# JokerYan/MS-GS

Measured on AMD Instinct MI355X. Metric: Mpixels/s fwd+bwd @1080p, 1M Gaussians; fraction of HBM roofline, higher is better.
Workload: dtype f32

## Files before the change

### ms-gs_amd/csrc/preprocess.hip

```cpp
#include "msgs_internal.h"

#include <type_traits>

#pragma clang fp contract(off)

namespace msgs {

namespace {

constexpr float SH_C0 = 0.28209479177387814f;
constexpr float SH_C1 = 0.4886025119029199f;
__device__ constexpr float SH_C2[5] = {1.0925484305920792f, -1.0925484305920792f, 0.31539156525252005f,
                                       -1.0925484305920792f, 0.5462742152960396f};
__device__ constexpr float SH_C3[7] = {-0.5900435899266435f, 2.890611442640554f, -0.4570457994644658f,
                                       0.3731763325901154f, -0.4570457994644658f, 1.445305721320277f,
                                       -0.5900435899266435f};

struct Cam {
    float V[16];
    float M[16];
    float cam[3];
};

__device__ __forceinline__ void load_cam(const ViewParams& vp, Cam& c) {
// ... 99 lines not shown
    float r = SH_C0 * S(0);
    if (deg > 0) {
        r = r - SH_C1 * y * S(1) + SH_C1 * z * S(2) - SH_C1 * x * S(3);
        if (deg > 1) {
            const float xx = x * x, yy = y * y, zz = z * z, xy = x * y, yz = y * z, xz = x * z;
            r = r + SH_C2[0] * xy * S(4) + SH_C2[1] * yz * S(5) + SH_C2[2] * (2.0f * zz - xx - yy) * S(6) +
                SH_C2[3] * xz * S(7) + SH_C2[4] * (xx - yy) * S(8);
            if (deg > 2) {
                r = r + SH_C3[0] * y * (3.0f * xx - yy) * S(9) + SH_C3[1] * xy * z * S(10) +
                    SH_C3[2] * y * (4.0f * zz - xx - yy) * S(11) +
                    SH_C3[3] * z * (2.0f * zz - 3.0f * xx - 3.0f * yy) * S(12) +
                    SH_C3[4] * x * (4.0f * zz - xx - yy) * S(13) + SH_C3[5] * z * (xx - yy) * S(14) +
                    SH_C3[6] * x * (xx - 3.0f * yy) * S(15);
            }
        }
    }
    return r;
}


__device__ __forceinline__ void sh_basis(int deg, float x, float y, float z, float b[16]) {
#pragma unroll
    for (int k = 0; k < 16; ++k) b[k] = 0.f;
    b[0] = SH_C0;
    if (deg > 0) {
        b[1] = -(SH_C1 * y); b[2] = SH_C1 * z; b[3] = -(SH_C1 * x);
        if (deg > 1) {
            const float xx = x * x, yy = y * y, zz = z * z, xy = x * y, yz = y * z, xz = x * z;
            b[4] = SH_C2[0] * xy; b[5] = SH_C2[1] * yz; b[6] = SH_C2[2] * (2.0f * zz - xx - yy);
            b[7] = SH_C2[3] * xz; b[8] = SH_C2[4] * (xx - yy);
            if (deg > 2) {
                b[9] = SH_C3[0] * y * (3.0f * xx - yy); b[10] = SH_C3[1] * xy * z;
                b[11] = SH_C3[2] * y * (4.0f * zz - xx - yy);
                b[12] = SH_C3[3] * z * (2.0f * zz - 3.0f * xx - 3.0f * yy);
                b[13] = SH_C3[4] * x * (4.0f * zz - xx - yy); b[14] = SH_C3[5] * z * (xx - yy);
                b[15] = SH_C3[6] * x * (xx - 3.0f * yy);
            }
        }
    }
}

__device__ __forceinline__ void wave_lds_fence() {
    __builtin_amdgcn_fence(__ATOMIC_RELEASE, "wavefront");
    __builtin_amdgcn_wave_barrier();
    __builtin_amdgcn_fence(__ATOMIC_ACQUIRE, "wavefront");
}

constexpr int ROW_F = 48;
constexpr int ROW_LDS = 49;
constexpr int K9_STAGE_ROWS = 32;

__device__ __forceinline__ int sh_row_float4s(int deg) { return deg == 0 ? 1 : deg == 1 ? 3 : deg == 2 ? 7 : 12; }

__device__ __forceinline__ void coop_load_rows(float* lds_rows, const float* g_rows, const uint8_t* idx, int nrow,
                                               int n4, int lane, int row0 = 0) {
    const int rpi = 64 / n4;
    const int sub = lane / n4, c = lane - sub * n4;
    for (int it = 0; it * rpi < nrow; ++it) {
        const int slot = it * rpi + sub;
        if (sub < rpi && slot < nrow) {
            const int sl = idx[slot];
            const float4 v = *reinterpret_cast<const float4*>(g_rows + (size_t)sl * ROW_F + 4 * c);
            float* d = lds_rows + (sl - row0) * ROW_LDS + 4 * c;
            d[0] = v.x; d[1] = v.y; d[2] = v.z; d[3] = v.w;
        }
    }
}

constexpr int HALF_F4 = 6;
constexpr int HALF_LDS = 25;
__device__ __forceinline__ void coop_load_rows_part(float* lds_rows, const float* g_rows, const uint8_t* idx, int nrow,
                                                    int f4_first, int n4, int lane) {
    const int rpi = 64 / n4;
    const int sub = lane / n4, c = lane - sub * n4;
    for (int it = 0; it * rpi < nrow; ++it) {
        const int slot = it * rpi + sub;
        if (sub < rpi && slot < nrow) {
            const int sl = idx[slot];
            const float4 v = *reinterpret_cast<const float4*>(g_rows + (size_t)sl * ROW_F + 4 * (f4_first + c));
            float* d = lds_rows + sl * HALF_LDS + 4 * c;
            d[0] = v.x; d[1] = v.y; d[2] = v.z; d[3] = v.w;
        }
    }
}

__device__ __forceinline__ void coop_store_rows(const float* lds_rows, float* g_rows, int nrow, uint64_t live,
                                                int nfloat, int lane, bool acc) {
    constexpr int n4 = ROW_F / 4, rpi = 64 / n4;
    const int sub = lane / n4, c = lane - sub * n4;
    for (int it = 0; it * rpi < nrow; ++it) {
        const int row = it * rpi + sub;
        if (sub < rpi && row < nrow) {
            const bool on = (live >> row) & 1ull;
            if (acc && !on) continue;
            float4 v = make_float4(0.f, 0.f, 0.f, 0.f);
            if (on) {
                const float* sp = lds_rows + row * ROW_LDS + 4 * c;
                v.x = 4 * c + 0 < nfloat ? sp[0] : 0.f;
                v.y = 4 * c + 1 < nfloat ? sp[1] : 0.f;
                v.z = 4 * c + 2 < nfloat ? sp[2] : 0.f;
                v.w = 4 * c + 3 < nfloat ? sp[3] : 0.f;
            }
            float4* dst = reinterpret_cast<float4*>(g_rows + (size_t)row * ROW_F + 4 * c);
            if (acc) { const float4 o = *dst; v.x = o.x + v.x; v.y = o.y + v.y; v.z = o.z + v.z; v.w = o.w + v.w; }
            *dst = v;
        }
    }
}

constexpr int REST_F = 45;

__device__ __forceinline__ float act_opacity(const msgs_gaussians_t& g, int i) {
    const float x = g.opacities[i];
    return g.raw_params == 1 ? 1.0f / (1.0f + expf(-x)) : x;
}
__device__ __forceinline__ void act_scales(const msgs_gaussians_t& g, int i, float* s) {
#pragma unroll
    for (int k = 0; k < 3; ++k) { const float x = g.scales[3 * i + k]; s[k] = g.raw_params == 1 ? expf(x) : x; }
}
__device__ __forceinline__ float act_rotation(const msgs_gaussians_t& g, int i, float* q) {
    const float4 q4 = reinterpret_cast<const float4*>(g.rotations)[i];
    q[0] = q4.x; q[1] = q4.y; q[2] = q4.z; q[3] = q4.w;
    if (g.raw_params == 0) return 1.0f;
    if (g.raw_params == 2) {
        const float4 r4 = reinterpret_cast<const float4*>(g.rotations_raw)[i];
        return sqrtf(r4.x * r4.x + r4.y * r4.y + r4.z * r4.z + r4.w * r4.w);
    }
    const float rn = sqrtf(q[0] * q[0] + q[1] * q[1] + q[2] * q[2] + q[3] * q[3]);
    const float n = fmaxf(rn, 1e-12f);
#pragma unroll
    for (int k = 0; k < 4; ++k) q[k] = q[k] / n;
    return rn;
}
__device__ __forceinline__ void normalize_backward(const float* q, float rn, float* dq) {
    const float n = fmaxf(rn, 1e-12f);
    const float dotq = rn < 1e-12f ? 0.f : q[0] * dq[0] + q[1] * dq[1] + q[2] * dq[2] + q[3] * dq[3];
#pragma unroll
    for (int k = 0; k < 4; ++k) dq[k] = (dq[k] - q[k] * dotq) / n;
}

typedef float msgs_f3 __attribute__((ext_vector_type(3)));
typedef msgs_f3 __attribute__((aligned(4))) msgs_f3_u;
__device__ __forceinline__ void coop_load_split_half_listed(float* lds_rows, const float* dc, const float* rest, int wave_first,
                                                            const uint8_t* idx, int nlisted, int half, int lane) {
    const int sub = lane >> 3, c = lane & 7;
    for (int it = 0; it * 8 < nlisted; ++it) {
        const int slot = it * 8 + sub;
        if (slot < nlisted) {
            const int sl = idx[slot];
            const size_t gi = (size_t)wave_first + sl;
            float* d = lds_rows + sl * HALF_LDS + 3 * c;
            const float* src = (half == 0 && c == 0) ? dc + gi * 3 : rest + gi * 45 + 3 * (8 * half + c - 1);
            const msgs_f3 v = *reinterpret_cast<const msgs_f3_u*>(src);
            d[0] = v.x; d[1] = v.y; d[2] = v.z;
        }
    }
}

__device__ __forceinline__ void coop_load_split_rows_listed(float* lds_rows, const float* dc, const float* rest, int wave_first,
                                                            const uint8_t* idx, int nlisted, int lane, int row0) {
    const int sub = lane >> 4, c = lane & 15;
    for (int it = 0; it * 4 < nlisted; ++it) {
        const int slot = it * 4 + sub;
        if (slot < nlisted) {
            const int sl = idx[slot];
            const size_t gi = (size_t)wave_first + sl;
            float* d = lds_rows + (sl - row0) * ROW_LDS + 3 * c;
            const float* src = c == 0 ? dc + gi * 3 : rest + gi * REST_F + 3 * (c - 1);
            const msgs_f3 v = *reinterpret_cast<const msgs_f3_u*>(src);
            d[0] = v.x; d[1] = v.y; d[2] = v.z;
        }
    }
}

__device__ __forceinline__ void coop_load_split_rows(float* lds_rows, const float* dc, const float* rest, int i,
                                                     bool in_range, int wave_first, int nrow, int lane, int lrow) {
    if (in_range) {
#pragma unroll
        for (int c = 0; c < 3; ++c) lds_rows[lrow * ROW_LDS + c] = dc[3 * (size_t)i + c];
    }
    const float* src = rest + (size_t)wave_first * REST_F;
    const int nflat = nrow * REST_F;
    for (int base = 0; base < nflat; base += 256) {
        const int f0 = base + lane * 4;
        float v[4] = {0.f, 0.f, 0.f, 0.f};
        if (f0 + 3 < nflat) {
            const float4 t = *reinterpret_cast<const float4*>(src + f0);
            v[0] = t.x; v[1] = t.y; v[2] = t.z; v[3] = t.w;
        } else {
#pragma unroll
            for (int j = 0; j < 4; ++j) if (f0 + j < nflat) v[j] = src[f0 + j];
        }
#pragma unroll
        for (int j = 0; j < 4; ++j) {
            const int f = f0 + j;
            if (f < nflat) { const int row = f / REST_F; lds_rows[row * ROW_LDS + 3 + (f - row * REST_F)] = v[j]; }
        }
    }
}

__device__ __forceinline__ void coop_store_split_rows(const float* lds_rows, float* d_dc, float* d_rest, int i,
                                                      bool in_range, int wave_first, int nrow, uint64_t live,
                                                      int nfloat, int lane, int lrow, bool acc = false) {
    if (in_range) {
        const bool on = (live >> lrow) & 1ull;
        if (!acc) {
#pragma unroll
            for (int c = 0; c < 3; ++c) d_dc[3 * (size_t)i + c] = on ? lds_rows[lrow * ROW_LDS + c] : 0.f;
        } else if (on) {
#pragma unroll
            for (int c = 0; c < 3; ++c) d_dc[3 * (size_t)i + c] = d_dc[3 * (size_t)i + c] + lds_rows[lrow * ROW_LDS + c];
        }
    }
    float* dst = d_rest + (size_t)wave_first * REST_F;
    const int nflat = nrow * REST_F;
    for (int base = 0; base < nflat; base += 256) {
        const int f0 = base + lane * 4;
        float v[4];
        bool on[4];
#pragma unroll
        for (int j = 0; j < 4; ++j) {
            const int f = min(f0 + j, nflat - 1);
            const int row = f / REST_F, k = f - row * REST_F;
            on[j] = (live >> row) & 1ull;
            v[j] = (on[j] && 3 + k < nfloat) ? lds_rows[row * ROW_LDS + 3 + k] : 0.f;
        }
        if (f0 + 3 < nflat) {
            float4* d4 = reinterpret_cast<float4*>(dst + f0);
            if (!acc) {
                *d4 = make_float4(v[0], v[1], v[2], v[3]);
            } else if (on[0] || on[3]) {
                const float4 o = *d4;
                *d4 = make_float4(o.x + v[0], o.y + v[1], o.z + v[2], o.w + v[3]);
            }
        } else {
#pragma unroll
            for (int j = 0; j < 4; ++j)
                if (f0 + j < nflat) {
                    if (!acc) dst[f0 + j] = v[j];
                    else if (on[j]) dst[f0 + j] = dst[f0 + j] + v[j];
                }
        }
    }
}

__device__ __forceinline__ void coop_adam_split_rows(const float* lds_rows, float* p_dc, float* p_rest, const AdamInBackward& ad,
                                                     int i, bool in_range, int wave_first, int nrow, uint64_t live,
                                                     int nfloat, int lane, int lrow) {
    if (in_range) {
        const bool on = (live >> lrow) & 1ull;
#pragma unroll
        for (int c = 0; c < 3; ++c) {
            const size_t at = 3 * (size_t)i + c;
            float p = p_dc[at], m = ad.m[1][at], v = ad.v[1][at];
            adam_update(p, on ? lds_rows[lrow * ROW_LDS + c] : 0.f, m, v, ad.nss[1], ad.a);
            p_dc[at] = p; ad.m[1][at] = m; ad.v[1][at] = v;
        }
    }
    const size_t off = (size_t)wave_first * REST_F;
    float* __restrict__ P = p_rest + off;
    float* __restrict__ M = ad.m[2] + off;
    float* __restrict__ V = ad.v[2] + off;
    const float nss = ad.nss[2];
    const int nflat = nrow * REST_F;
    for (int base = 0; base < nflat; base += 256) {
        const int f0 = base + lane * 4;
        float g[4];
#pragma unroll
        for (int j = 0; j < 4; ++j) {
            const int f = min(f0 + j, nflat - 1);
            const int row = f / REST_F, k = f - row * REST_F;
            g[j] = (((live >> row) & 1ull) && 3 + k < nfloat) ? lds_rows[row * ROW_LDS + 3 + k] : 0.f;
        }
        if (f0 + 3 < nflat) {
            float4 p = *reinterpret_cast<const float4*>(P + f0), m = *reinterpret_cast<const float4*>(M + f0),
                   v = *reinterpret_cast<const float4*>(V + f0);
            adam_update(p.x, g[0], m.x, v.x, nss, ad.a);
            adam_update(p.y, g[1], m.y, v.y, nss, ad.a);
            adam_update(p.z, g[2], m.z, v.z, nss, ad.a);
            adam_update(p.w, g[3], m.w, v.w, nss, ad.a);
            *reinterpret_cast<float4*>(P + f0) = p;
            *reinterpret_cast<float4*>(M + f0) = m;
            *reinterpret_cast<float4*>(V + f0) = v;
        } else {
#pragma unroll
            for (int j = 0; j < 4; ++j)
                if (f0 + j < nflat) {
                    float p = P[f0 + j], m = M[f0 + j], v = V[f0 + j];
                    adam_update(p, g[j], m, v, nss, ad.a);
                    P[f0 + j] = p; M[f0 + j] = m; V[f0 + j] = v;
                }
        }
    }
}

template <bool SPLIT_ROWS>
__global__ __launch_bounds__(256) void preprocess_kernel(ViewParams vp, msgs_gaussians_t g,
                                                         int32_t* __restrict__ radii,
                                                         float* __restrict__ pixel_sizes,
                                                         char* __restrict__ geom, ZeroJob zj,
                                                         uint32_t* __restrict__ heavy_list,
                                                         uint32_t* __restrict__ heavy_count,
                                                         uint32_t* __restrict__ heavy_blk, int write_litrec) {
    __shared__ float s_rows[4][64 * HALF_LDS];
    __shared__ uint8_t s_idx[4][64];
    __shared__ uint32_t s_heavy[4], s_hvw[4];
    const int P = g.P;
    {
        const size_t t0 = (size_t)blockIdx.x * blockDim.x + threadIdx.x, nt = (size_t)gridDim.x * blockDim.x;
        for (size_t t = t0; t < zj.n0; t += nt) zj.p0[t] = 0u;
        for (size_t t = t0; t < zj.n1; t += nt) zj.p1[t] = 0u;
    }
    const int i = blockIdx.x * blockDim.x + threadIdx.x;
    const int lane = threadIdx.x & 63, wv = threadIdx.x >> 6;
    const bool in_range = i < P;
    const GeomLayout L(P);
    GaussRec* rec = reinterpret_cast<GaussRec*>(geom + L.rec);
    BinRec* binrec = reinterpret_cast<BinRec*>(geom + L.binrec);
    uint32_t* tiles = reinterpret_cast<uint32_t*>(geom + L.tiles);
    uint32_t* key = reinterpret_cast<uint32_t*>(geom + L.key);
    uint32_t* flags = reinterpret_cast<uint32_t*>(geom + L.flags);
    float* weight = reinterpret_cast<float*>(geom + L.weight);

    Cam cm;
    load_cam(vp, cm);
// ... 144 lines not shown
            binrec[i].q1 = make_float4(sC, tau2, __uint_as_float((uint32_t)minx | ((uint32_t)miny << 16)),
                                       __uint_as_float((uint32_t)maxx | ((uint32_t)maxy << 16)));
            if (vp.cell_sx >= 0)
                out_cells = cell_range_pack(minx, miny, maxx, maxy, vp.cell_sx, vp.cell_sy) << TILE_COUNT_BITS;
        }
        out_radius = (int32_t)my_radius;
        out_tau2 = tau2;
        out_tiles = count;
        out_key = count ? __float_as_uint(t[2]) : 0xFFFFFFFFu;
        out_flags |= 8u;
        out_weight = w;
    }
    if (in_range) {
        radii[i] = out_radius;
        pixel_sizes[i] = out_psize;
        tiles[i] = out_tiles | out_cells;
        key[i] = out_key;
        flags[i] = out_flags;
        weight[i] = out_weight;
    }
    if (heavy_count) {
        const bool hv = out_tiles > OCC_HEAVY_MIN && out_tau2 > -1.0e38f;
        const uint64_t m = __ballot(hv);
        const size_t slot = (size_t)blockIdx.x * 4 + wv;
        if (hv) reinterpret_cast<uint2*>(heavy_list)[slot * 64 + __popcll(m & ((1ull << lane) - 1ull))] = make_uint2((uint32_t)i, out_key);
        uint32_t wmax = hv ? (uint32_t)(-__log2f(1.0f - fminf(0.99f, o_eff)) * 2048.0f) + 2u : 0u;
        for (int off = 32; off > 0; off >>= 1) wmax += (uint32_t)__shfl_xor((int)wmax, off);
        if (lane == 0) { heavy_count[slot] = (uint32_t)__popcll(m); s_heavy[wv] = (uint32_t)__popcll(m); s_hvw[wv] = wmax; }
        __syncthreads();
        if (threadIdx.x == 0)
            reinterpret_cast<uint2*>(heavy_blk)[blockIdx.x] = make_uint2(s_heavy[0] + s_heavy[1] + s_heavy[2] + s_heavy[3],
                                                                         min(s_hvw[0] + s_hvw[1] + s_hvw[2] + s_hvw[3], 0x0FFFFFFFu));
    }
}

__device__ __forceinline__ double (&camera_lds())[4][CAM_PARTIALS] {
    __shared__ double s[4][CAM_PARTIALS];
    return s;
}

__device__ __forceinline__ float (&camera_dir_lds())[3][256] {
    __shared__ float s[3][256];
    return s;
}

template <bool TEXTBOOK, bool ADAM, bool DEPTH = false, bool CAMERA = false>
__global__ __launch_bounds__(256) __attribute__((amdgpu_waves_per_eu(CAMERA ? 4 : 5))) void preprocess_backward_kernel(ViewParams vp, msgs_gaussians_t g,
                                                                  const int32_t* __restrict__ radii,
                                                                  const char* __restrict__ geom,
                                                                  const grad_acc_t* __restrict__ grad_rec,
                                                                  msgs_grads_t grads,
                                                                  std::conditional_t<CAMERA, CamPartials, AdamInBackward> ad) {
    static_assert(!(CAMERA && ADAM), "camera gradients are not offered with the optimizer step in the backward");
    __shared__ float s_rows[4][K9_STAGE_ROWS * ROW_LDS];
    __shared__ uint8_t s_idx[4][64];
    const int P = g.P;
    const int i = blockIdx.x * blockDim.x + threadIdx.x;
    const int lane = threadIdx.x & 63, wv = threadIdx.x >> 6;
    const bool in_range = i < P;
    const GeomLayout L(P);
    const uint32_t* flags = reinterpret_cast<const uint32_t*>(geom + L.flags);
    const int K = vp.sh_coeffs;
    const int deg = vp.sh_degree;

    float dmean[3] = {0.f, 0.f, 0.f};
    float g2x = 0.f, g2y = 0.f, dopac = 0.f;
    float dcov[6] = {0.f, 0.f, 0.f, 0.f, 0.f, 0.f};
    float dcolr[3] = {0.f, 0.f, 0.f};
    float dscale[3] = {0.f, 0.f, 0.f};
    float dq[4] = {0.f, 0.f, 0.f, 0.f};
    const bool rendered = in_range && radii[i] > 0;
    const bool raw = g.raw_params != 0;
    const bool split_in = raw && g.shs == nullptr;
    const bool staged_sh = raw || (g.shs != nullptr && grads.dL_dshs != nullptr && K == 16);
    const bool factored_sh = !ADAM && raw && grads.dL_dfeatures_dc == nullptr;
    const bool accum = !ADAM && grads.accumulate != 0;
    const int wave_first = blockIdx.x * blockDim.x + wv * 64;
    const uint64_t live = __ballot(rendered);
    if (staged_sh) {
        if (rendered) s_idx[wv][__popcll(live & ((1ull << lane) - 1ull))] = (uint8_t)lane;
    }
    uint32_t fl = 0;
    float p[3] = {0.f, 0.f, 0.f};
    float cdt[3] = {0.f, 0.f, 0.f}, cdh[3] = {0.f, 0.f, 0.f}, cjt[9] = {};

    if (rendered) {
        Cam cm;
        load_cam(vp, cm);
        float4 ga, gb, gc;
        if constexpr (TEXTBOOK) {
            const double* gr = reinterpret_cast<const double*>(grad_rec) + (size_t)i * (DEPTH ? DET_INST_FLOATS_DEPTH : 9);
            ga = make_float4((float)gr[0], (float)gr[1], (float)gr[2], (float)gr[3]);
            gb = make_float4((float)gr[4], (float)gr[5], (float)gr[6], (float)gr[7]);
            gc = make_float4((float)gr[8], DEPTH ? (float)gr[9] : 0.f, 0.f, 0.f);
        } else {
            const grad_acc_t* gr = grad_rec + (size_t)i * GRAD_REC_FLOATS;
            grad_acc_t t[GRAD_REC_FLOATS];
            typedef grad_acc_t acc2 __attribute__((ext_vector_type(2)));
#pragma unroll
            for (int k = 0; k < GRAD_REC_FLOATS / 2; ++k) {
                const acc2 v2 = reinterpret_cast<const acc2*>(gr)[k];
                t[2 * k] = v2.x; t[2 * k + 1] = v2.y;
            }
            ga = make_float4((float)t[0], (float)t[1], (float)t[2], (float)t[3]);
            gb = make_float4((float)t[4], (float)t[5], (float)t[6], (float)t[7]);
            gc = make_float4((float)t[8], DEPTH ? (float)t[9] : 0.f, 0.f, 0.f);
        }
        const float gA = TEXTBOOK ? ga.z : -0.5f * ga.z, gBh = TEXTBOOK ? ga.w : -0.5f * ga.w,
                    gC = TEXTBOOK ? gb.x : -0.5f * gb.x;
        const float o_in = act_opacity(g, i);
        if constexpr (TEXTBOOK)
            dopac = reinterpret_cast<const float*>(geom + L.weight)[i] * gb.y;
        else
            dopac = o_in > 0.f ? gb.y / o_in : 0.f;
        if (raw) dopac = dopac * (o_in * (1.0f - o_in));
        dcolr[0] = gb.z; dcolr[1] = gb.w; dcolr[2] = gc.x;
        fl = flags[i];
        p[0] = g.means3D[3 * i]; p[1] = g.means3D[3 * i + 1]; p[2] = g.means3D[3 * i + 2];

        float cov3D[6];
        float R[3][3], S[3] = {0.f, 0.f, 0.f};
        float qr = 0.f, qx = 0.f, qy = 0.f, qz = 0.f, qnorm = 1.0f;
        float sact[3] = {1.f, 1.f, 1.f};
        if (g.cov3D_precomp) {
#pragma unroll
            for (int k = 0; k < 6; ++k) cov3D[k] = g.cov3D_precomp[6 * i + k];
        } else {
            float s[3], q[4];
            act_scales(g, i, s);
            qnorm = act_rotation(g, i, q);
            qr = q[0]; qx = q[1]; qy = q[2]; qz = q[3];
            sact[0] = s[0]; sact[1] = s[1]; sact[2] = s[2];
            cov3d_from_scale_rot(s, vp.scale_modifier, q, cov3D);
            S[0] = vp.scale_modifier * s[0]; S[1] = vp.scale_modifier * s[1]; S[2] = vp.scale_modifier * s[2];
            R[0][0] = 1.f - 2.f * (qy * qy + qz * qz); R[0][1] = 2.f * (qx * qy - qr * qz); R[0][2] = 2.f * (qx * qz + qr * qy);
            R[1][0] = 2.f * (qx * qy + qr * qz); R[1][1] = 1.f - 2.f * (qx * qx + qz * qz); R[1][2] = 2.f * (qy * qz - qr * qx);
            R[2][0] = 2.f * (qx * qz - qr * qy); R[2][1] = 2.f * (qy * qz + qr * qx); R[2][2] = 1.f - 2.f * (qx * qx + qy * qy);
        }

        float t[3];
        view_point(cm.V, p, t);
        Cov2D c2;
        compute_cov2d(t, vp, cov3D, cm.V, c2);
        const float ca = c2.a, cb = c2.b, cc = c2.c;
        const float denom = ca * cc - cb * cb;
        if constexpr (TEXTBOOK) {
            g2x = ga.x; g2y = ga.y;
        } else {
            constexpr float KLOG = -0.72134752044448170368f;
            constexpr float LN2 = 0.69314718055994530942f;
            const float det_inv = 1.f / denom;
            const float sA = KLOG * (cc * det_inv), sBh = KLOG * (-cb * det_inv), sC = KLOG * (ca * det_inv);
            g2x = (sA * ga.x + sBh * ga.y) * (LN2 * vp.W);
            g2y = (sC * ga.y + sBh * ga.x) * (LN2 * vp.H);
        }
        const float denom2inv = 1.0f / ((denom * denom) + 0.0000001f);
        float dL_da = 0.f, dL_db = 0.f, dL_dc = 0.f;
        if (denom2inv != 0.f) {
            dL_da = denom2inv * (-cc * cc * gA + 2 * cb * cc * gBh + (denom - ca * cc) * gC);
            dL_dc = denom2inv * (-ca * ca * gC + 2 * ca * cb * gBh + (denom - ca * cc) * gA);
            dL_db = denom2inv * 2 * (cb * cc * gA - (denom + 2 * cb * cb) * gBh + ca * cb * gC);
            const float(*T)[3] = c2.T;
            dcov[0] = T[0][0] * T[0][0] * dL_da + T[0][0] * T[1][0] * dL_db + T[1][0] * T[1][0] * dL_dc;
            dcov[3] = T[0][1] * T[0][1] * dL_da + T[0][1] * T[1][1] * dL_db + T[1][1] * T[1][1] * dL_dc;
            dcov[5] = T[0][2] * T[0][2] * dL_da + T[0][2] * T[1][2] * dL_db + T[1][2] * T[1][2] * dL_dc;
            dcov[1] = 2 * T[0][0] * T[0][1] * dL_da + (T[0][0] * T[1][1] + T[0][1] * T[1][0]) * dL_db + 2 * T[1][0] * T[1][1] * dL_dc;
            dcov[2] = 2 * T[0][0] * T[0][2] * dL_da + (T[0][0] * T[1][2] + T[0][2] * T[1][0]) * dL_db + 2 * T[1][0] * T[1][2] * dL_dc;
            dcov[4] = 2 * T[0][2] * T[0][1] * dL_da + (T[0][1] * T[1][2] + T[0][2] * T[1][1]) * dL_db + 2 * T[1][1] * T[1][2] * dL_dc;
        }
        {
            const float Sg[3][3] = {{cov3D[0], cov3D[1], cov3D[2]}, {cov3D[1], cov3D[3], cov3D[4]},
                                    {cov3D[2], cov3D[4], cov3D[5]}};
            float ST0[3], ST1[3], dT0[3], dT1[3];
#pragma unroll
            for (int k = 0; k < 3; ++k) {
                ST0[k] = Sg[k][0] * c2.T[0][0] + Sg[k][1] * c2.T[0][1] + Sg[k][2] * c2.T[0][2];
                ST1[k] = Sg[k][0] * c2.T[1][0] + Sg[k][1] * c2.T[1][1] + Sg[k][2] * c2.T[1][2];
            }
#pragma unroll
            for (int k = 0; k < 3; ++k) {
                dT0[k] = 2 * ST0[k] * dL_da + ST1[k] * dL_db;
                dT1[k] = 2 * ST1[k] * dL_dc + ST0[k] * dL_db;
            }
// ... 56 lines not shown
                dscale[j] = vp.scale_modifier * ds;
#pragma unroll
                for (int a = 0; a < 3; ++a) dR[a][j] = dM[a][j] * S[j];
            }
            const float r = qr, x = qx, y = qy, z = qz;
            dq[0] = 2.f * (-z * dR[0][1] + y * dR[0][2] + z * dR[1][0] - x * dR[1][2] - y * dR[2][0] + x * dR[2][1]);
            dq[1] = 2.f * (y * dR[0][1] + z * dR[0][2] + y * dR[1][0] - 2.f * x * dR[1][1] - r * dR[1][2] + z * dR[2][0] + r * dR[2][1] - 2.f * x * dR[2][2]);
            dq[2] = 2.f * (-2.f * y * dR[0][0] + x * dR[0][1] + r * dR[0][2] + x * dR[1][0] + z * dR[1][2] - r * dR[2][0] + z * dR[2][1] - 2.f * y * dR[2][2]);
            dq[3] = 2.f * (-2.f * z * dR[0][0] - r * dR[0][1] + x * dR[0][2] + r * dR[1][0] - 2.f * z * dR[1][1] + y * dR[1][2] + x * dR[2][0] + y * dR[2][1]);
            if (raw) {
#pragma unroll
                for (int j = 0; j < 3; ++j) dscale[j] = dscale[j] * sact[j];
                const float qv[4] = {r, x, y, z};
                normalize_backward(qv, qnorm, dq);
            }
        }
    }
    if constexpr (CAMERA) {
        double(&s_cam)[4][CAM_PARTIALS] = camera_lds();
        float* F = s_rows[wv];
        if (live != 0) {
#pragma unroll
            for (int k = 0; k < 3; ++k) {
                F[(0 + k) * 64 + lane] = p[k];
                F[(3 + k) * 64 + lane] = cdt[k];
                F[(6 + k) * 64 + lane] = cdh[k];
            }
#pragma unroll
            for (int k = 0; k < 9; ++k) F[(9 + k) * 64 + lane] = cjt[k];
            wave_lds_fence();
            const int m = lane % 24, half = lane / 24;
            const int j = (m % 12) / 3, k = m % 3;
            const float* fa = F + (m < 12 ? 3 + k : 6 + k) * 64;
            const float* fp = F + (j < 3 ? j : 0) * 64;
            const float* fj = F + (9 + 3 * (j < 3 ? j : 0) + k) * 64;
            const bool pj = j < 3, wj = m < 12 && j < 3;
            double acc = 0.0;
            if (half < 2) {
                const int l0 = 32 * half;
#pragma unroll 8
                for (int l = l0; l < l0 + 32; ++l) {
                    const float a = fa[l], b = fp[l], c = fj[l];
                    acc += (pj ? (double)b : 1.0) * (double)a + (wj ? (double)c : 0.0);
                }
            }
            const double other = __shfl(acc, (lane + 24) & 63);
            if (lane < 24) s_cam[wv][lane] = acc + other;
        } else if (lane < 24) {
            s_cam[wv][lane] = 0.0;
        }
        float(&s_dir)[3][256] = camera_dir_lds();
        s_dir[0][threadIdx.x] = 0.f; s_dir[1][threadIdx.x] = 0.f; s_dir[2][threadIdx.x] = 0.f;
    }
    auto colour_backward = [&](const float* sh, float* dsh) {
        {
#pragma unroll
            for (int c = 0; c < 3; ++c)
                if (fl & (1u << c)) dcolr[c] = 0.f;
            const float dox = p[0] - vp.campos[0], doy = p[1] - vp.campos[1], doz = p[2] - vp.campos[2];
            const float len = sqrtf(dox * dox + doy * doy + doz * doz);
            const float x = dox / len, y = doy / len, z = doz / len;
            float ddir[3] = {0.f, 0.f, 0.f};
            auto coef = [&](int k, float basis, float bx, float by, float bz) {
                float s = 0.f;
#pragma unroll
                for (int c = 0; c < 3; ++c) {
                    const float shv = sh[k * 3 + c];
                    if (dsh) dsh[k * 3 + c] = basis * dcolr[c];
                    s += shv * dcolr[c];
                }
                ddir[0] += bx * s; ddir[1] += by * s; ddir[2] += bz * s;
            };
            coef(0, SH_C0, 0.f, 0.f, 0.f);
            if (deg > 0) {
                coef(1, -SH_C1 * y, 0.f, -SH_C1, 0.f);
                coef(2, SH_C1 * z, 0.f, 0.f, SH_C1);
                coef(3, -SH_C1 * x, -SH_C1, 0.f, 0.f);
                if (deg > 1) {
                    const float xx = x * x, yy = y * y, zz = z * z, xy = x * y, yz = y * z, xz = x * z;
                    coef(4, SH_C2[0] * xy, SH_C2[0] * y, SH_C2[0] * x, 0.f);
                    coef(5, SH_C2[1] * yz, 0.f, SH_C2[1] * z, SH_C2[1] * y);
                    coef(6, SH_C2[2] * (2.f * zz - xx - yy), SH_C2[2] * -2.f * x, SH_C2[2] * -2.f * y, SH_C2[2] * 4.f * z);
                    coef(7, SH_C2[3] * xz, SH_C2[3] * z, 0.f, SH_C2[3] * x);
                    coef(8, SH_C2[4] * (xx - yy), SH_C2[4] * 2.f * x, SH_C2[4] * -2.f * y, 0.f);
                    if (deg > 2) {
                        coef(9, SH_C3[0] * y * (3.f * xx - yy), SH_C3[0] * 6.f * xy, SH_C3[0] * (3.f * xx - 3.f * yy), 0.f);
                        coef(10, SH_C3[1] * xy * z, SH_C3[1] * yz, SH_C3[1] * xz, SH_C3[1] * xy);
                        coef(11, SH_C3[2] * y * (4.f * zz - xx - yy), SH_C3[2] * -2.f * xy, SH_C3[2] * (4.f * zz - xx - 3.f * yy), SH_C3[2] * 8.f * yz);
                        coef(12, SH_C3[3] * z * (2.f * zz - 3.f * xx - 3.f * yy), SH_C3[3] * -6.f * xz, SH_C3[3] * -6.f * yz, SH_C3[3] * (6.f * zz - 3.f * xx - 3.f * yy));
                        coef(13, SH_C3[4] * x * (4.f * zz - xx - yy), SH_C3[4] * (4.f * zz - 3.f * xx - yy), SH_C3[4] * -2.f * xy, SH_C3[4] * 8.f * xz);
                        coef(14, SH_C3[5] * z * (xx - yy), SH_C3[5] * 2.f * xz, SH_C3[5] * -2.f * yz, SH_C3[5] * (xx - yy));
                        coef(15, SH_C3[6] * x * (xx - 3.f * yy), SH_C3[6] * (3.f * xx - 3.f * yy), SH_C3[6] * -6.f * xy, 0.f);
                    }
                }
            }
            const int ncoef = (deg + 1) * (deg + 1);
            if (dsh && !staged_sh)
                for (int k = ncoef; k < K; ++k) { dsh[k * 3] = 0.f; dsh[k * 3 + 1] = 0.f; dsh[k * 3 + 2] = 0.f; }
            const float dotv = x * ddir[0] + y * ddir[1] + z * ddir[2];
            dmean[0] += (ddir[0] - x * dotv) / len;
            dmean[1] += (ddir[1] - y * dotv) / len;
            dmean[2] += (ddir[2] - z * dotv) / len;
            if constexpr (CAMERA) {
                float(&s_dir)[3][256] = camera_dir_lds();
                s_dir[0][threadIdx.x] = (ddir[0] - x * dotv) / len;
                s_dir[1][threadIdx.x] = (ddir[1] - y * dotv) / len;
                s_dir[2][threadIdx.x] = (ddir[2] - z * dotv) / len;
            }
        }
    };
    const bool do_colour = !g.colors_precomp;
    if (do_colour && staged_sh) {
        const int nfloat = 3 * (deg + 1) * (deg + 1);
#pragma unroll 1
        for (int h = 0; h < 64 / K9_STAGE_ROWS; ++h) {
            const int row0 = h * K9_STAGE_ROWS;
            const int first = wave_first + row0;
            const int nrow = min(K9_STAGE_ROWS, P - first);
            if (nrow <= 0) break;
            const uint64_t live_h = (live >> row0) & ((1ull << K9_STAGE_ROWS) - 1ull);
            const bool mine = (lane / K9_STAGE_ROWS) == h;
            const int lrow = lane - row0;
            wave_lds_fence();
            if (split_in) {
                if (live_h != 0)
                    coop_load_split_rows_listed(s_rows[wv], g.features_dc, g.features_rest, wave_first,
                                                s_idx[wv] + __popcll(live & ((1ull << row0) - 1ull)), __popcll(live_h), lane, row0);
            } else {
                coop_load_rows(s_rows[wv], g.shs + (size_t)wave_first * ROW_F,
                               s_idx[wv] + __popcll(live & ((1ull << row0) - 1ull)), __popcll(live_h), sh_row_float4s(deg),
                               lane, row0);
            }
            wave_lds_fence();
            if (rendered && mine) {
                float* row = &s_rows[wv][lrow * ROW_LDS];
                colour_backward(row, factored_sh ? nullptr : row);
            }
            if (factored_sh) continue;
            wave_lds_fence();
            if constexpr (ADAM)
                coop_adam_split_rows(s_rows[wv], const_cast<float*>(g.features_dc), const_cast<float*>(g.features_rest), ad, i,
                                     in_range && mine, first, nrow, live_h, nfloat, lane, lrow);
            else if (raw)
                coop_store_split_rows(s_rows[wv], grads.dL_dfeatures_dc, grads.dL_dfeatures_rest, i, in_range && mine, first,
                                      nrow, live_h, nfloat, lane, lrow, accum);
            else
                coop_store_rows(s_rows[wv], grads.dL_dshs + (size_t)first * ROW_F, nrow, live_h, nfloat, lane, accum);
        }
    } else if (do_colour) {
        float* dsh = grads.dL_dshs && in_range ? grads.dL_dshs + (size_t)3 * K * i : nullptr;
        if (rendered) colour_backward(g.shs + (size_t)3 * K * i, dsh);
        else if (dsh) for (int k = 0; k < 3 * K; ++k) dsh[k] = 0.f;
    }
    if constexpr (CAMERA) {
        double(&s_cam)[4][CAM_PARTIALS] = camera_lds();
        float(&s_dir)[3][256] = camera_dir_lds();
        const bool any = live != 0 && do_colour;
        wave_lds_fence();
#pragma unroll
        for (int k = 0; k < 3; ++k) {
            const double v = any ? -wave_sum_f64((double)s_dir[k][threadIdx.x]) : 0.0;
            if (lane == 0) s_cam[wv][24 + k] = v;
        }
        __syncthreads();
        if (threadIdx.x < CAM_PARTIALS) {
            const int m = threadIdx.x;
            ad.rows[(size_t)blockIdx.x * CAM_ROW + m] = ((s_cam[0][m] + s_cam[1][m]) + s_cam[2][m]) + s_cam[3][m];
        }
    }
    if (!in_range) return;

    if (grads.dL_dmeans2D) { grads.dL_dmeans2D[3 * i] = g2x; grads.dL_dmeans2D[3 * i + 1] = g2y; grads.dL_dmeans2D[3 * i + 2] = 0.f; }
    if constexpr (ADAM) {
        auto step3 = [&](const float* param, int t, const float* gr) {
            float* P = const_cast<float*>(param) + 3 * (size_t)i;
            float* M = ad.m[t] + 3 * (size_t)i;
            float* V = ad.v[t] + 3 * (size_t)i;
#pragma unroll
            for (int c = 0; c < 3; ++c) {
                float pp = P[c], mm = M[c], vv = V[c];
                adam_update(pp, gr[c], mm, vv, ad.nss[t], ad.a);
                P[c] = pp; M[c] = mm; V[c] = vv;
            }
        };
        step3(g.means3D, 0, dmean);
        {
            float* P = const_cast<float*>(g.opacities) + i;
            float pp = *P, mm = ad.m[3][i], vv = ad.v[3][i];
            adam_update(pp, dopac, mm, vv, ad.nss[3], ad.a);
            *P = pp; ad.m[3][i] = mm; ad.v[3][i] = vv;
        }
        step3(g.scales, 4, dscale);
        {
            float4* P = reinterpret_cast<float4*>(const_cast<float*>(g.rotations)) + i;
            float4* M = reinterpret_cast<float4*>(ad.m[5]) + i;
            float4* V = reinterpret_cast<float4*>(ad.v[5]) + i;
            float4 pp = *P, mm = *M, vv = *V;
            adam_update(pp.x, dq[0], mm.x, vv.x, ad.nss[5], ad.a);
            adam_update(pp.y, dq[1], mm.y, vv.y, ad.nss[5], ad.a);
            adam_update(pp.z, dq[2], mm.z, vv.z, ad.nss[5], ad.a);
// ... 47 lines not shown
    if (i >= P) return;
    float c0 = 0.f, c1 = 0.f, c2 = 0.f;
    if (radii[i] > 0) {
        const GeomLayout L(P);
        const uint32_t fl = reinterpret_cast<const uint32_t*>(geom + L.flags)[i];
        const grad_acc_t* gr = grad_rec + (size_t)i * rec_stride;
        c0 = (fl & 1u) ? 0.f : (float)gr[6];
        c1 = (fl & 2u) ? 0.f : (float)gr[7];
        c2 = (fl & 4u) ? 0.f : (float)gr[8];
    }
    dL_dcolors[3 * (size_t)i] = c0; dL_dcolors[3 * (size_t)i + 1] = c1; dL_dcolors[3 * (size_t)i + 2] = c2;
}

__global__ __launch_bounds__(256) void sh_grad_from_views_kernel(int P, int n_views, int deg,
                                                                 const float* __restrict__ means3D,
                                                                 const float* __restrict__ campos,
                                                                 int64_t cs,
                                                                 const float* __restrict__ drgb,
                                                                 int64_t ds, float scale, float* __restrict__ d_dc,
                                                                 float* __restrict__ d_rest) {
    __shared__ float s_rows[4][64 * ROW_LDS];
    const int i = blockIdx.x * blockDim.x + threadIdx.x;
    const int lane = threadIdx.x & 63, wv = threadIdx.x >> 6;
    const bool in_range = i < P;
    const int wave_first = blockIdx.x * blockDim.x + wv * 64;
    float acc[48];
#pragma unroll
    for (int k = 0; k < 48; ++k) acc[k] = 0.f;
    if (in_range) {
        const float p[3] = {means3D[3 * i], means3D[3 * i + 1], means3D[3 * i + 2]};
        for (int v = 0; v < n_views; ++v) {
            const float* d = drgb + (size_t)v * ds + (size_t)i * 3;
            const float* cp = campos + (size_t)v * cs;
            const float d0 = d[0], d1 = d[1], d2 = d[2];
            if (d0 == 0.f && d1 == 0.f && d2 == 0.f) continue;
            const float dox = p[0] - cp[0], doy = p[1] - cp[1], doz = p[2] - cp[2];
            const float len = sqrtf(dox * dox + doy * doy + doz * doz);
            float b[16];
            sh_basis(deg, dox / len, doy / len, doz / len, b);
#pragma unroll
            for (int k = 0; k < 16; ++k) {
                acc[3 * k] = acc[3 * k] + b[k] * d0;
                acc[3 * k + 1] = acc[3 * k + 1] + b[k] * d1;
                acc[3 * k + 2] = acc[3 * k + 2] + b[k] * d2;
            }
        }
    }
    float* row = &s_rows[wv][lane * ROW_LDS];
#pragma unroll
    for (int k = 0; k < 48; ++k) row[k] = acc[k] * scale;
    wave_lds_fence();
    const int nrow = min(64, P - wave_first);
    if (nrow > 0)
        coop_store_split_rows(s_rows[wv], d_dc, d_rest, i, in_range, wave_first, nrow, ~0ull, 48, lane, lane);
}

constexpr int CAM_FINISH_THREADS = 1024;
constexpr int CAM_SUM_GROUPS = 64;
__global__ __launch_bounds__(CAM_FINISH_THREADS) void camera_finish_kernel(const double* __restrict__ rows, int nrows, int chunk,
                                                                            double* __restrict__ out, float* __restrict__ dV,
                                                                            float* __restrict__ dPM, float* __restrict__ dcp) {
    constexpr int PAIRS = CAM_ROW / 2, GROUPS = CAM_FINISH_THREADS / PAIRS, U = 16;
    __shared__ double2 s_sum[GROUPS][PAIRS];
    const int q = threadIdx.x % PAIRS, grp = threadIdx.x / PAIRS;
    const int first = blockIdx.x * chunk, n = min(chunk, nrows - first);
    const double2* r2 = reinterpret_cast<const double2*>(rows) + (size_t)first * PAIRS;
    double2 acc = make_double2(0.0, 0.0);
    int r = grp;
    for (; r + (U - 1) * GROUPS < n; r += U * GROUPS) {
        double2 v[U];
#pragma unroll
        for (int u = 0; u < U; ++u) v[u] = r2[(size_t)(r + u * GROUPS) * PAIRS + q];
#pragma unroll
        for (int u = 0; u < U; ++u) { acc.x += v[u].x; acc.y += v[u].y; }
    }
    for (; r < n; r += GROUPS) {
        const double2 v = r2[(size_t)r * PAIRS + q];
        acc.x += v.x; acc.y += v.y;
    }
    s_sum[grp][q] = acc;
    __syncthreads();
#pragma unroll
    for (int h = GROUPS / 2; h > 0; h >>= 1) {
        if (grp < h) {
            const double2 o = s_sum[grp + h][q];
            s_sum[grp][q] = make_double2(s_sum[grp][q].x + o.x, s_sum[grp][q].y + o.y);
        }
        __syncthreads();
    }
    if (out) {
        if (threadIdx.x < PAIRS) reinterpret_cast<double2*>(out)[(size_t)blockIdx.x * PAIRS + threadIdx.x] = s_sum[0][threadIdx.x];
        return;
    }
    if (threadIdx.x >= 35) return;
    const int t = threadIdx.x;
    auto total = [&](int m) { return (float)((m & 1) ? s_sum[0][m >> 1].y : s_sum[0][m >> 1].x); };
    if (t < 16) {
        const int j = t >> 2, k = t & 3;
        if (dV) dV[t] = k < 3 ? total(3 * j + k) : 0.f;
    } else if (t < 32) {
        const int f = t - 16, j = f >> 2, k = f & 3;
        if (dPM) dPM[f] = k == 2 ? 0.f : total(12 + 3 * j + (k == 3 ? 2 : k));
    } else if (dcp) {
        dcp[t - 32] = total(24 + (t - 32));
    }
}

// ... 112 lines not shown
```

Baseline: 1959.

## Stage SH rows via async global-to-LDS DMA issued before geometry backward

The preprocess backward now fetches spherical-harmonic rows into LDS with global_load_lds DMA in contiguous blocks, replacing the compacted index-listed per-lane loads. The first half-wave stage is issued before the geometry backward math so the transfer overlaps with it. Parameter loads (opacity, scales, rotations) are hoisted earlier. Split dc/rest inputs keep their native layouts in LDS, and the store and Adam helpers gain explicit leading dimensions. This trades some over-fetch of dead rows and manual waitcnt management for fewer dependent load latencies.

```diff
diff --git a/ms-gs_amd/csrc/preprocess.hip b/ms-gs_amd/csrc/preprocess.hip
--- a/ms-gs_amd/csrc/preprocess.hip
+++ b/ms-gs_amd/csrc/preprocess.hip
@@ -175,21 +175,6 @@
 
 __device__ __forceinline__ int sh_row_float4s(int deg) { return deg == 0 ? 1 : deg == 1 ? 3 : deg == 2 ? 7 : 12; }
 
-__device__ __forceinline__ void coop_load_rows(float* lds_rows, const float* g_rows, const uint8_t* idx, int nrow,
-                                               int n4, int lane, int row0 = 0) {
-    const int rpi = 64 / n4;
-    const int sub = lane / n4, c = lane - sub * n4;
-    for (int it = 0; it * rpi < nrow; ++it) {
-        const int slot = it * rpi + sub;
-        if (sub < rpi && slot < nrow) {
-            const int sl = idx[slot];
-            const float4 v = *reinterpret_cast<const float4*>(g_rows + (size_t)sl * ROW_F + 4 * c);
-            float* d = lds_rows + (sl - row0) * ROW_LDS + 4 * c;
-            d[0] = v.x; d[1] = v.y; d[2] = v.z; d[3] = v.w;
-        }
-    }
-}
-
 constexpr int HALF_F4 = 6;
 constexpr int HALF_LDS = 25;
 __device__ __forceinline__ void coop_load_rows_part(float* lds_rows, const float* g_rows, const uint8_t* idx, int nrow,
@@ -207,6 +192,7 @@
     }
 }
 
+template <int RS = ROW_LDS>
 __device__ __forceinline__ void coop_store_rows(const float* lds_rows, float* g_rows, int nrow, uint64_t live,
                                                 int nfloat, int lane, bool acc) {
     constexpr int n4 = ROW_F / 4, rpi = 64 / n4;
@@ -218,7 +204,7 @@
             if (acc && !on) continue;
             float4 v = make_float4(0.f, 0.f, 0.f, 0.f);
             if (on) {
-                const float* sp = lds_rows + row * ROW_LDS + 4 * c;
+                const float* sp = lds_rows + row * RS + 4 * c;
                 v.x = 4 * c + 0 < nfloat ? sp[0] : 0.f;
                 v.y = 4 * c + 1 < nfloat ? sp[1] : 0.f;
                 v.z = 4 * c + 2 < nfloat ? sp[2] : 0.f;
@@ -233,27 +219,83 @@
 
 constexpr int REST_F = 45;
 
-__device__ __forceinline__ float act_opacity(const msgs_gaussians_t& g, int i) {
-    const float x = g.opacities[i];
+constexpr int K9_ROW_SLOTS = ROW_F / 4 + 1;
+constexpr int K9_ROW_LDS = 4 * K9_ROW_SLOTS;
+constexpr int K9_SPLIT_REST = 3 * K9_STAGE_ROWS;
+#define MSGS_AS1 __attribute__((address_space(1)))
+#define MSGS_AS3 __attribute__((address_space(3)))
+__device__ __forceinline__ void k9_fetch16(float* lds, const float* src, bool dma, int lane) {
+    if (dma) {
+        __builtin_amdgcn_global_load_lds((const MSGS_AS1 void*)src, (MSGS_AS3 void*)(uintptr_t)lds, 16, 0, 0);
+    } else {
+        float* d = lds + 4 * lane;
+#pragma unroll
+        for (int t = 0; t < 4; ++t) d[t] = src[t];
+    }
+}
+__device__ __forceinline__ void k9_fetch_rows(float* lds, const float* shs, int first, uint32_t live_h, int nfloat, int lane) {
+    const bool dma = ((uintptr_t)shs & 15) == 0;
+    const int n4 = (nfloat + 3) >> 2;
+    constexpr int n_inst = (K9_STAGE_ROWS * K9_ROW_SLOTS + 63) / 64;
+#pragma unroll 1
+    for (int it = 0; it < n_inst; ++it) {
+        const int slot = it * 64 + lane;
+        const int r = slot / K9_ROW_SLOTS, c = slot - r * K9_ROW_SLOTS;
+        if (r < K9_STAGE_ROWS && c < n4 && ((live_h >> r) & 1u))
+            k9_fetch16(lds + it * 256, shs + ((size_t)first + r) * ROW_F + 4 * c, dma, lane);
+    }
+}
+template <int ROWF>
+__device__ __forceinline__ void k9_fetch_block(float* lds, const float* src, int nrow, uint32_t live_h, int k0, int nfloat,
+                                               int lane) {
+    const bool dma = ((uintptr_t)src & 15) == 0;
+    constexpr int n_inst = (K9_STAGE_ROWS * ROWF / 4 + 63) / 64;
+    const int nvalid = nrow * ROWF;
+#pragma unroll 1
+    for (int it = 0; it < n_inst; ++it) {
+        const int f = 4 * (it * 64 + lane);
+        if (f >= K9_STAGE_ROWS * ROWF) continue;
+        const int ra = f / ROWF, rb = (f + 3) / ROWF;
+        const bool need = (((live_h >> ra) & 1u) && k0 + (f - ra * ROWF) < nfloat) ||
+                          (rb != ra && ((live_h >> rb) & 1u) && k0 < nfloat);
+        if (!need) continue;
+        if (f + 3 < nvalid) {
+            k9_fetch16(lds + it * 256, src + f, dma, lane);
+        } else {
+#pragma unroll
+            for (int t = 0; t < 3; ++t)
+                if (f + t < nvalid) lds[f + t] = src[f + t];
+        }
+    }
+}
+
+__device__ __forceinline__ float act_opacity_of(const msgs_gaussians_t& g, float x) {
     return g.raw_params == 1 ? 1.0f / (1.0f + expf(-x)) : x;
 }
+__device__ __forceinline__ float act_opacity(const msgs_gaussians_t& g, int i) { return act_opacity_of(g, g.opacities[i]); }
+__device__ __forceinline__ void act_scales_of(const msgs_gaussians_t& g, const float* x, float* s) {
+#pragma unroll
+    for (int k = 0; k < 3; ++k) s[k] = g.raw_params == 1 ? expf(x[k]) : x[k];
+}
 __device__ __forceinline__ void act_scales(const msgs_gaussians_t& g, int i, float* s) {
-#pragma unroll
-    for (int k = 0; k < 3; ++k) { const float x = g.scales[3 * i + k]; s[k] = g.raw_params == 1 ? expf(x) : x; }
+    const float x[3] = {g.scales[3 * i], g.scales[3 * i + 1], g.scales[3 * i + 2]};
+    act_scales_of(g, x, s);
+}
+__device__ __forceinline__ float act_rotation_of(const msgs_gaussians_t& g, const float4 q4, const float4 r4, float* q) {
+    q[0] = q4.x; q[1] = q4.y; q[2] = q4.z; q[3] = q4.w;
+    if (g.raw_params == 0) return 1.0f;
+    if (g.raw_params == 2)
+        return sqrtf(r4.x * r4.x + r4.y * r4.y + r4.z * r4.z + r4.w * r4.w);
+    const float rn = sqrtf(q[0] * q[0] + q[1] * q[1] + q[2] * q[2] + q[3] * q[3]);
+    const float n = fmaxf(rn, 1e-12f);
+#pragma unroll
+    for (int k = 0; k < 4; ++k) q[k] = q[k] / n;
+    return rn;
 }
 __device__ __forceinline__ float act_rotation(const msgs_gaussians_t& g, int i, float* q) {
     const float4 q4 = reinterpret_cast<const float4*>(g.rotations)[i];
-    q[0] = q4.x; q[1] = q4.y; q[2] = q4.z; q[3] = q4.w;
-    if (g.raw_params == 0) return 1.0f;
-    if (g.raw_params == 2) {
-        const float4 r4 = reinterpret_cast<const float4*>(g.rotations_raw)[i];
-        return sqrtf(r4.x * r4.x + r4.y * r4.y + r4.z * r4.z + r4.w * r4.w);
-    }
-    const float rn = sqrtf(q[0] * q[0] + q[1] * q[1] + q[2] * q[2] + q[3] * q[3]);
-    const float n = fmaxf(rn, 1e-12f);
-#pragma unroll
-    for (int k = 0; k < 4; ++k) q[k] = q[k] / n;
-    return rn;
+    const float4 r4 = g.raw_params == 2 ? reinterpret_cast<const float4*>(g.rotations_raw)[i] : q4;
+    return act_rotation_of(g, q4, r4, q);
 }
 __device__ __forceinline__ void normalize_backward(const float* q, float rn, float* dq) {
     const float n = fmaxf(rn, 1e-12f);
@@ -280,22 +322,6 @@
     }
 }
 
-__device__ __forceinline__ void coop_load_split_rows_listed(float* lds_rows, const float* dc, const float* rest, int wave_first,
-                                                            const uint8_t* idx, int nlisted, int lane, int row0) {
-    const int sub = lane >> 4, c = lane & 15;
-    for (int it = 0; it * 4 < nlisted; ++it) {
-        const int slot = it * 4 + sub;
-        if (slot < nlisted) {
-            const int sl = idx[slot];
-            const size_t gi = (size_t)wave_first + sl;
-            float* d = lds_rows + (sl - row0) * ROW_LDS + 3 * c;
-            const float* src = c == 0 ? dc + gi * 3 : rest + gi * REST_F + 3 * (c - 1);
-            const msgs_f3 v = *reinterpret_cast<const msgs_f3_u*>(src);
-            d[0] = v.x; d[1] = v.y; d[2] = v.z;
-        }
-    }
-}
-
 __device__ __forceinline__ void coop_load_split_rows(float* lds_rows, const float* dc, const float* rest, int i,
                                                      bool in_range, int wave_first, int nrow, int lane, int lrow) {
     if (in_range) {
@@ -322,17 +348,18 @@
     }
 }
 
-__device__ __forceinline__ void coop_store_split_rows(const float* lds_rows, float* d_dc, float* d_rest, int i,
+__device__ __forceinline__ void coop_store_split_rows(const float* lds_dc, int dc_ld, const float* lds_rest, int rest_ld,
+                                                      float* d_dc, float* d_rest, int i,
                                                       bool in_range, int wave_first, int nrow, uint64_t live,
                                                       int nfloat, int lane, int lrow, bool acc = false) {
     if (in_range) {
         const bool on = (live >> lrow) & 1ull;
         if (!acc) {
 #pragma unroll
-            for (int c = 0; c < 3; ++c) d_dc[3 * (size_t)i + c] = on ? lds_rows[lrow * ROW_LDS + c] : 0.f;
+            for (int c = 0; c < 3; ++c) d_dc[3 * (size_t)i + c] = on ? lds_dc[lrow * dc_ld + c] : 0.f;
         } else if (on) {
 #pragma unroll
-            for (int c = 0; c < 3; ++c) d_dc[3 * (size_t)i + c] = d_dc[3 * (size_t)i + c] + lds_rows[lrow * ROW_LDS + c];
+            for (int c = 0; c < 3; ++c) d_dc[3 * (size_t)i + c] = d_dc[3 * (size_t)i + c] + lds_dc[lrow * dc_ld + c];
         }
     }
     float* dst = d_rest + (size_t)wave_first * REST_F;
@@ -346,7 +373,7 @@
             const int f = min(f0 + j, nflat - 1);
             const int row = f / REST_F, k = f - row * REST_F;
             on[j] = (live >> row) & 1ull;
-            v[j] = (on[j] && 3 + k < nfloat) ? lds_rows[row * ROW_LDS + 3 + k] : 0.f;
+            v[j] = (on[j] && 3 + k < nfloat) ? lds_rest[row * rest_ld + k] : 0.f;
         }
         if (f0 + 3 < nflat) {
             float4* d4 = reinterpret_cast<float4*>(dst + f0);
@@ -367,7 +394,8 @@
     }
 }
 
-__device__ __forceinline__ void coop_adam_split_rows(const float* lds_rows, float* p_dc, float* p_rest, const AdamInBackward& ad,
+__device__ __forceinline__ void coop_adam_split_rows(const float* lds_dc, int dc_ld, const float* lds_rest, int rest_ld,
+                                                     float* p_dc, float* p_rest, const AdamInBackward& ad,
                                                      int i, bool in_range, int wave_first, int nrow, uint64_t live,
                                                      int nfloat, int lane, int lrow) {
     if (in_range) {
@@ -376,7 +404,7 @@
         for (int c = 0; c < 3; ++c) {
             const size_t at = 3 * (size_t)i + c;
             float p = p_dc[at], m = ad.m[1][at], v = ad.v[1][at];
-            adam_update(p, on ? lds_rows[lrow * ROW_LDS + c] : 0.f, m, v, ad.nss[1], ad.a);
+            adam_update(p, on ? lds_dc[lrow * dc_ld + c] : 0.f, m, v, ad.nss[1], ad.a);
             p_dc[at] = p; ad.m[1][at] = m; ad.v[1][at] = v;
         }
     }
@@ -393,7 +421,7 @@
         for (int j = 0; j < 4; ++j) {
             const int f = min(f0 + j, nflat - 1);
             const int row = f / REST_F, k = f - row * REST_F;
-            g[j] = (((live >> row) & 1ull) && 3 + k < nfloat) ? lds_rows[row * ROW_LDS + 3 + k] : 0.f;
+            g[j] = (((live >> row) & 1ull) && 3 + k < nfloat) ? lds_rest[row * rest_ld + k] : 0.f;
         }
         if (f0 + 3 < nflat) {
             float4 p = *reinterpret_cast<const float4*>(P + f0), m = *reinterpret_cast<const float4*>(M + f0),
@@ -644,8 +672,7 @@
                                                                   msgs_grads_t grads,
                                                                   std::conditional_t<CAMERA, CamPartials, AdamInBackward> ad) {
     static_assert(!(CAMERA && ADAM), "camera gradients are not offered with the optimizer step in the backward");
-    __shared__ float s_rows[4][K9_STAGE_ROWS * ROW_LDS];
-    __shared__ uint8_t s_idx[4][64];
+    __shared__ __attribute__((aligned(16))) float s_rows[4][K9_STAGE_ROWS * K9_ROW_LDS];
     const int P = g.P;
     const int i = blockIdx.x * blockDim.x + threadIdx.x;
     const int lane = threadIdx.x & 63, wv = threadIdx.x >> 6;
@@ -669,16 +696,36 @@
     const bool accum = !ADAM && grads.accumulate != 0;
     const int wave_first = blockIdx.x * blockDim.x + wv * 64;
     const uint64_t live = __ballot(rendered);
-    if (staged_sh) {
-        if (rendered) s_idx[wv][__popcll(live & ((1ull << lane) - 1ull))] = (uint8_t)lane;
+    Cam cm;
+    if constexpr (!CAMERA) load_cam(vp, cm);
+    const bool do_colour = !g.colors_precomp;
+    auto fetch_run = [&](int h) {
+        int lane_f = lane;
+        asm volatile("" : "+v"(lane_f));
+        const int row0 = h * K9_STAGE_ROWS;
+        const int first = __builtin_amdgcn_readfirstlane(wave_first + row0);
+        const uint32_t live_h = (uint32_t)(live >> row0);
+        const int nfloat = 3 * (deg + 1) * (deg + 1);
+        if (live_h == 0) return;
+        if (split_in) {
+            const int nrow = min(K9_STAGE_ROWS, P - first);
+            k9_fetch_block<3>(s_rows[wv], g.features_dc + (size_t)first * 3, nrow, live_h, 0, nfloat, lane_f);
+            if (deg > 0)
+                k9_fetch_block<REST_F>(s_rows[wv] + K9_SPLIT_REST, g.features_rest + (size_t)first * REST_F, nrow, live_h, 3,
+                                       nfloat, lane_f);
+        } else {
+            k9_fetch_rows(s_rows[wv], g.shs, first, live_h, nfloat, lane_f);
+        }
+    };
+    if constexpr (!CAMERA) {
+        if (do_colour && staged_sh) fetch_run(0);
     }
     uint32_t fl = 0;
     float p[3] = {0.f, 0.f, 0.f};
     float cdt[3] = {0.f, 0.f, 0.f}, cdh[3] = {0.f, 0.f, 0.f}, cjt[9] = {};
 
     if (rendered) {
-        Cam cm;
-        load_cam(vp, cm);
+        if constexpr (CAMERA) load_cam(vp, cm);
         float4 ga, gb, gc;
         if constexpr (TEXTBOOK) {
             const double* gr = reinterpret_cast<const double*>(grad_rec) + (size_t)i * (DEPTH ? DET_INST_FLOATS_DEPTH : 9);
@@ -691,6 +738,7 @@
             typedef grad_acc_t acc2 __attribute__((ext_vector_type(2)));
 #pragma unroll
             for (int k = 0; k < GRAD_REC_FLOATS / 2; ++k) {
+                if (2 * k + 1 > (DEPTH ? 9 : 8)) { t[2 * k] = 2 * k <= (DEPTH ? 9 : 8) ? gr[2 * k] : (grad_acc_t)0; t[2 * k + 1] = (grad_acc_t)0; continue; }
                 const acc2 v2 = reinterpret_cast<const acc2*>(gr)[k];
                 t[2 * k] = v2.x; t[2 * k + 1] = v2.y;
             }
@@ -698,19 +746,28 @@
             gb = make_float4((float)t[4], (float)t[5], (float)t[6], (float)t[7]);
             gc = make_float4((float)t[8], DEPTH ? (float)t[9] : 0.f, 0.f, 0.f);
         }
+        const float o_raw = g.opacities[i];
+        fl = flags[i];
+        p[0] = g.means3D[3 * i]; p[1] = g.means3D[3 * i + 1]; p[2] = g.means3D[3 * i + 2];
+        float cov3D[6];
+        float s_raw[3];
+        float4 q4, r4;
+        if (!g.cov3D_precomp) {
+#pragma unroll
+            for (int k = 0; k < 3; ++k) s_raw[k] = g.scales[3 * i + k];
+            q4 = reinterpret_cast<const float4*>(g.rotations)[i];
+            if constexpr (!CAMERA) { if (g.raw_params == 2) r4 = reinterpret_cast<const float4*>(g.rotations_raw)[i]; }
+        }
         const float gA = TEXTBOOK ? ga.z : -0.5f * ga.z, gBh = TEXTBOOK ? ga.w : -0.5f * ga.w,
                     gC = TEXTBOOK ? gb.x : -0.5f * gb.x;
-        const float o_in = act_opacity(g, i);
+        const float o_in = act_opacity_of(g, o_raw);
         if constexpr (TEXTBOOK)
             dopac = reinterpret_cast<const float*>(geom + L.weight)[i] * gb.y;
         else
             dopac = o_in > 0.f ? gb.y / o_in : 0.f;
         if (raw) dopac = dopac * (o_in * (1.0f - o_in));
         dcolr[0] = gb.z; dcolr[1] = gb.w; dcolr[2] = gc.x;
-        fl = flags[i];
-        p[0] = g.means3D[3 * i]; p[1] = g.means3D[3 * i + 1]; p[2] = g.means3D[3 * i + 2];
-
-        float cov3D[6];
+
         float R[3][3], S[3] = {0.f, 0.f, 0.f};
         float qr = 0.f, qx = 0.f, qy = 0.f, qz = 0.f, qnorm = 1.0f;
         float sact[3] = {1.f, 1.f, 1.f};
@@ -719,8 +776,9 @@
             for (int k = 0; k < 6; ++k) cov3D[k] = g.cov3D_precomp[6 * i + k];
         } else {
             float s[3], q[4];
-            act_scales(g, i, s);
-            qnorm = act_rotation(g, i, q);
+            act_scales_of(g, s_raw, s);
+            if constexpr (CAMERA) { if (g.raw_params == 2) r4 = reinterpret_cast<const float4*>(g.rotations_raw)[i]; }
+            qnorm = act_rotation_of(g, q4, r4, q);
             qr = q[0]; qx = q[1]; qy = q[2]; qz = q[3];
             sact[0] = s[0]; sact[1] = s[1]; sact[2] = s[2];
             cov3d_from_scale_rot(s, vp.scale_modifier, q, cov3D);
@@ -883,7 +941,7 @@
         float(&s_dir)[3][256] = camera_dir_lds();
         s_dir[0][threadIdx.x] = 0.f; s_dir[1][threadIdx.x] = 0.f; s_dir[2][threadIdx.x] = 0.f;
     }
-    auto colour_backward = [&](const float* sh, float* dsh) {
+    auto colour_backward = [&](const float* sh, float* dsh, int rest_delta = 0) {
         {
 #pragma unroll
             for (int c = 0; c < 3; ++c)
@@ -896,8 +954,9 @@
                 float s = 0.f;
 #pragma unroll
                 for (int c = 0; c < 3; ++c) {
-                    const float shv = sh[k * 3 + c];
-                    if (dsh) dsh[k * 3 + c] = basis * dcolr[c];
+                    const int at = k * 3 + c + (k ? rest_delta : 0);
+                    const float shv = sh[at];
+                    if (dsh) dsh[at] = basis * dcolr[c];
                     s += shv * dcolr[c];
                 }
                 ddir[0] += bx * s; ddir[1] += by * s; ddir[2] += bz * s;
@@ -940,9 +999,10 @@
             }
         }
     };
-    const bool do_colour = !g.colors_precomp;
     if (do_colour && staged_sh) {
         const int nfloat = 3 * (deg + 1) * (deg + 1);
+        const int dc_ld = split_in ? 3 : K9_ROW_LDS, rest_ld = split_in ? REST_F : K9_ROW_LDS;
+        const int rest_at = split_in ? K9_SPLIT_REST : 3;
 #pragma unroll 1
         for (int h = 0; h < 64 / K9_STAGE_ROWS; ++h) {
             const int row0 = h * K9_STAGE_ROWS;
@@ -952,31 +1012,28 @@
             const uint64_t live_h = (live >> row0) & ((1ull << K9_STAGE_ROWS) - 1ull);
             const bool mine = (lane / K9_STAGE_ROWS) == h;
             const int lrow = lane - row0;
-            wave_lds_fence();
-            if (split_in) {
-                if (live_h != 0)
-                    coop_load_split_rows_listed(s_rows[wv], g.features_dc, g.features_rest, wave_first,
-                                                s_idx[wv] + __popcll(live & ((1ull << row0) - 1ull)), __popcll(live_h), lane, row0);
-            } else {
-                coop_load_rows(s_rows[wv], g.shs + (size_t)wave_first * ROW_F,
-                               s_idx[wv] + __popcll(live & ((1ull << row0) - 1ull)), __popcll(live_h), sh_row_float4s(deg),
-                               lane, row0);
-            }
+            if (CAMERA || h > 0) {
+                wave_lds_fence();
+                asm volatile("s_waitcnt lgkmcnt(0)" ::: "memory");
+                fetch_run(h);
+            }
+            asm volatile("s_waitcnt vmcnt(0)" ::: "memory");
             wave_lds_fence();
             if (rendered && mine) {
-                float* row = &s_rows[wv][lrow * ROW_LDS];
-                colour_backward(row, factored_sh ? nullptr : row);
+                float* row = &s_rows[wv][lrow * dc_ld];
+                colour_backward(row, factored_sh ? nullptr : row, rest_at - 3 + lrow * (rest_ld - dc_ld));
             }
             if (factored_sh) continue;
             wave_lds_fence();
             if constexpr (ADAM)
-                coop_adam_split_rows(s_rows[wv], const_cast<float*>(g.features_dc), const_cast<float*>(g.features_rest), ad, i,
-                                     in_range && mine, first, nrow, live_h, nfloat, lane, lrow);
+                coop_adam_split_rows(s_rows[wv], dc_ld, s_rows[wv] + rest_at, rest_ld, const_cast<float*>(g.features_dc),
+                                     const_cast<float*>(g.features_rest), ad, i, in_range && mine, first, nrow, live_h, nfloat,
+                                     lane, lrow);
             else if (raw)
-                coop_store_split_rows(s_rows[wv], grads.dL_dfeatures_dc, grads.dL_dfeatures_rest, i, in_range && mine, first,
-                                      nrow, live_h, nfloat, lane, lrow, accum);
+                coop_store_split_rows(s_rows[wv], dc_ld, s_rows[wv] + rest_at, rest_ld, grads.dL_dfeatures_dc,
+                                      grads.dL_dfeatures_rest, i, in_range && mine, first, nrow, live_h, nfloat, lane, lrow, accum);
             else
-                coop_store_rows(s_rows[wv], grads.dL_dshs + (size_t)first * ROW_F, nrow, live_h, nfloat, lane, accum);
+                coop_store_rows<K9_ROW_LDS>(s_rows[wv], grads.dL_dshs + (size_t)first * ROW_F, nrow, live_h, nfloat, lane, accum);
         }
     } else if (do_colour) {
         float* dsh = grads.dL_dshs && in_range ? grads.dL_dshs + (size_t)3 * K * i : nullptr;
@@ -1130,7 +1187,8 @@
     wave_lds_fence();
     const int nrow = min(64, P - wave_first);
     if (nrow > 0)
-        coop_store_split_rows(s_rows[wv], d_dc, d_rest, i, in_range, wave_first, nrow, ~0ull, 48, lane, lane);
+        coop_store_split_rows(s_rows[wv], ROW_LDS, s_rows[wv] + 3, ROW_LDS, d_dc, d_rest, i, in_range, wave_first, nrow, ~0ull, 48,
+                              lane, lane);
 }
 
 constexpr int CAM_FINISH_THREADS = 1024;
```

Result: no change. 1971, median of 6 (+0.7%).
